# makezur/super_primitive

Measured on AMD Instinct MI355X. Metric: GN iters/sec (640x480x64-seg frame pairs), higher is better.
Workload: dtype f32; 1 GPU; Replica-shaped two-frame SfM, 640x480, 64 segments (grid, 4 px overlap), pyramid level 0 of a 3-level pyramid; BASELINE.json configs[1]; pairs_per_gpu=384, segment_pixels_per_pair=373056, optimiser=gn, tile_points=8192, span_points=4096, granule=64

## Files before the change

include/sp_hip.h:

```cpp
#ifndef SP_HIP_H
#define SP_HIP_H

#include <stdint.h>

#ifdef __cplusplus
extern "C" {
#endif

#define SP_ABI_VERSION 17

#define SP_EINVAL (-1)
#define SP_ELIMIT (-2)

#define SP_GRAD_PARTIAL_FLOATS 16
#define SP_GN_PARTIAL_FLOATS   32
#define SP_GNA_PARTIAL_FLOATS  48

int sp_abi_version(void);


int sp_mask_count(const uint8_t* masks, int N, int H, int W, int32_t* row_counts, int32_t* counts,
                  int32_t* seg_off, void* stream);

int sp_table_fill(const uint8_t* masks, const float* logdepth, const float* keypoints, int N, int H, int W,
// ... 113 lines not shown
#define SP_COST_WAVE_SPANS 0x100
#define SP_COST_DEPTH_TABLE 0x200

int sp_pairs_cost(const SpPair* pairs, const int32_t* chunks, const int32_t* spans, int n_spans, int mode, float irls_eps,
                  float* span_partials, float* seg_partials, void* stream);

int sp_pairs_adam_step(const SpPair* pairs, int n_pairs, int max_N, const float* span_partials, const float* seg_partials,
                       float lr_kld, float lr_pose, float lr_aff, float* state, float* losses, void* stream);

#define SP_LM_STATE_FLOATS 8
int sp_pairs_gn_step(const SpPair* pairs, int n_pairs, int max_N, const float* span_partials, const float* seg_partials,
                     float lm_up, float lm_down, float lm_min, float* lm_state, float* backup, float* costs, void* stream);

int sp_pairs_cost_active(const SpPair* pairs, const int32_t* chunks, const int32_t* spans, int n_spans, int mode, float irls_eps,
                         float* span_partials, float* seg_partials, const int32_t* done, void* stream);
int sp_pairs_gn_step_conv(const SpPair* pairs, int n_pairs, int max_N, const float* span_partials, const float* seg_partials,
                          float lm_up, float lm_down, float lm_min, float* lm_state, float* backup, float* costs, float conv_tol,
                          int32_t* done, void* stream);

#define SP_MAX_PHASES 12
#define SP_PHASE_POSE_ONLY 1
#define SP_PHASE_WAVE_SPANS 2
#define SP_PHASE_DEPTH_TABLE 4
#define SP_PHASE_DEPTH_DAMP_SHIFT 8
#define SP_PHASE_DEPTH_DAMP(k) (((k) & 0xff) << SP_PHASE_DEPTH_DAMP_SHIFT)
#define SP_PHASE_ADAM 8
#define SP_PHASE_PREDICTED_EXIT 16
typedef struct SpPhase {
    const SpPair* pairs;
    const int32_t* chunks;
// ... 272 lines not shown
```

super_primitive_amd/_lib.py:

```python
from __future__ import annotations

import ctypes
import os
from ctypes import c_float, c_int, c_void_p

_HERE = os.path.dirname(os.path.abspath(__file__))
LIB_PATH = os.environ.get("SP_HIP_LIB") or os.path.join(_HERE, "csrc", "libsp_hip.so")

P = c_void_p
I = c_int
F = c_float

SIGNATURES = {
    "sp_abi_version": [],
    "sp_mask_count": [P, I, I, I, P, P, P, P],
    "sp_table_fill": [P, P, P, I, I, I, P, P, P, P, P, P],
    "sp_table_sample_source": [P, P, P, P, P, I, I, I, I, P, I, I, P, P, I, P],
    "sp_pack_rgb": [P, I, I, I, P, P],
    "sp_blur_decimate": [P, I, I, I, P, P],
    "sp_photo_cost_grad": [P, P, P, P, P, P, I, I, I, I, I, P, P, P, I, I, P, P, I, P, P, F, P, P, P, P, P, P],
    "sp_points_workspace_floats": [I, I],
    "sp_points_cost_grad": [P, P, I, I, I, I, P, I, I, P, P, I, P, P, F, P, P, P, P, P],
    "sp_photo_stats": [P, P, P, P, I, I, I, I, P, P, P, I, I, P, P, I, P, P, F, P, P, P, P, P, P, P, P, I, P],
    "sp_pairs_cost": [P, P, P, I, I, F, P, P, P],
    "sp_pairs_adam_step": [P, I, I, P, P, F, F, F, P, P, P],
    "sp_pairs_gn_step": [P, I, I, P, P, F, F, F, P, P, P, P],
    "sp_pairs_cost_active": [P, P, P, I, I, F, P, P, P, P],
    "sp_pairs_gn_step_conv": [P, I, I, P, P, F, F, F, P, P, P, F, P, P],
    "sp_prepare_count": [P, I, I, I, P],
    "sp_prepare_count_boxed": [P, I, I, I, P],
    "sp_prepare_fill": [P, I, I, I, P],
    "sp_prepare_sample": [P, I, I, P],
    "sp_prepare_sample_pairs": [P, I, P, I, I, P],
    "sp_prepare_blur": [P, I, I, I, P],
    "sp_prepare_pack": [P, I, I, P],
    "sp_prepare_blur_pack": [P, I, I, P],
    "sp_prepare_gather": [P, P, I, P, P],
    "sp_host_work_list_chunks": [P, I, I, I],
    "sp_host_layout": [P, I, I, P, I, I, P, P, P, P, P],
    "sp_host_work_list": [P, P, P, I, I, I, I, I, P, P, P, P, P, P],
    "sp_pairs_schedule_cost": [P, P, P],
    "sp_pairs_schedule_gn_step": [P, I, I, F, F, F, P, P, P, P, P, P, P],
# ... 253 lines not shown
```

super_primitive_amd/csrc/sp_cost.hip:

```cpp
#include "sp_solve_device.h"

namespace {

struct TileCtx {
    gptr_u32 pix;
    gptr_f4 src4;
    gptr_f32 trg;
    Cam Ks;
    Warp w;
    float shift;
    float gain, bias;
    float ax, ay;
    uint32_t row_bytes;
    int Wl, Hl;
    int start, count;
};

struct Geo {
    float qx, qy, qz;
    float zinv, zi;
    float px, py, pz;
};

struct Pending {
// ... 239 lines not shown
    f32x2 hd01;
    f32x2 hd[2];
    float h11;
    f32x2 D, bd;
    float cost, n;
    float cost_mark, n_mark;
};

struct Pending2 {
    f32x2 qxy; float qz, zinv, zi;
    f32x2 wxy; float m;
    f32x2 srg; float sb;
    uint32_t off0;
};

template <bool DT = false>
__device__ __forceinline__ void prepare2(const TileCtx& c, const PairConsts& k, float shift, uint32_t pw, const f32x4 s, Pending2& p) {
    const f32x2 colrow{(float)(pw & 0xffffu), (float)((pw >> 16) & 0x7fffu)};
    const bool src_ok = (int32_t)pw < 0;
    const float d = DT ? s.w * shift : fast_exp(s.w + shift);
    const f32x2 xy = pfma(colrow, k.ifxy, k.nKc) * d;
    const f32x2 qxy = pfma(k.R03, f32x2{xy.x, xy.x}, pfma(k.R14, f32x2{xy.y, xy.y}, pfma(k.R25, f32x2{d, d}, k.t01)));
    const float qz = fmaf(k.R6, xy.x, fmaf(k.R7, xy.y, fmaf(k.R8, d, k.t2)));
    const bool zguard = fabsf(qz) > 1e-6f;
    const float zinv = zguard ? __builtin_amdgcn_rcpf(qz) : 1e-6f;
    const f32x2 uv = qxy * k.Kf * zinv + k.Ktc;
    const f32x2 n = pfma(uv, k.invWH, f32x2{-1.f, -1.f});
    const bool ok = (fabsf(n.x) <= 0.99f) && (fabsf(n.y) <= 0.99f) && (qz > k.zmin) && src_ok && (d > 1e-7f);
    p.m = ok ? 1.f : 0.f;
    p.qxy = qxy; p.qz = qz;
    p.zinv = ok ? zinv : 0.f;
    p.zi = (ok && zguard) ? zinv : 0.f;
    p.srg = f32x2{s.x, s.y}; p.sb = s.z;
    const f32x2 ixy = pfma(n, k.sxy, k.sxy);
    const f32x2 fl{floorf(ixy.x), floorf(ixy.y)};
// ... 170 lines not shown
        float v[10] = {A.hd01.x, A.hd01.y, A.hd[0].x, A.hd[0].y, A.hd[1].x, A.hd[1].y, A.D.x + A.D.y, A.bd.x + A.bd.y,
                       A.cost - A.cost_mark, A.n - A.n_mark};
        wave_sum_to_lanes<10>(v, lane, pos, ok);
        if (ok) store_partial<WT>(rec + pos, v[0]);
        A.cost_mark = A.cost; A.n_mark = A.n;
    }
    const f32x2 z{0.f, 0.f};
    A.hd01 = z; A.hd[0] = z; A.hd[1] = z; A.D = z; A.bd = z;
}

__device__ __forceinline__ uint32_t pix_from_colour_bits(const f32x4 s) {
    const uint32_t a = __builtin_bit_cast(uint32_t, s.x), b = __builtin_bit_cast(uint32_t, s.y), c = __builtin_bit_cast(uint32_t, s.z);
    const uint32_t v = (a & 0x7fu) | ((b & 0x7fu) << 7) | ((c & 0x3fu) << 14);
    return (v & 0x3ffu) | (((v >> 10) & 0x1ffu) << 16) | ((v >> 19) << 31);
}
template <int ABL, bool WT, bool AFF = false, bool W64 = false>
__device__ __forceinline__ void run_span_gn(const TileCtx& c, const SpPair& pr, const int4* __restrict__ chunks, int q0,
                                            int n_chunks, int total, float irls_eps, float* __restrict__ span_rec,
                                            float* __restrict__ seg_partials, float* lds) {
    constexpr int TRIP = W64 ? 64 : SP_BLOCK;
    constexpr bool DT = ABL == 6;
    constexpr int NV = AFF ? SP_GNA_PARTIAL_FLOATS : SP_GN_PARTIAL_FLOATS, NS = AFF ? SP_GNA_SEG_FLOATS : SP_GN_SEG_FLOATS;
    GnAcc A;
    AffAcc AA;
    MixA ma{f32x2{0.f, 0.f}, f32x2{0.f, 0.f}};
    {
        const f32x2 z{0.f, 0.f};
        AA.haa = AA.hab = AA.hbb = AA.ba = AA.bb = AA.hda = AA.hdb = 0.f;
        AA.pa01 = z; AA.pb01 = z; AA.pa[0] = z; AA.pa[1] = z; AA.pb[0] = z; AA.pb[1] = z;
    }
    {
        const f32x2 z{0.f, 0.f};
        A.h00 = z; A.bp01 = z; A.hd01 = z;
#pragma unroll
// ... 16 lines not shown
        kc.t01 = f32x2{w.t[0], w.t[1]};        kc.Kf = sgpr2(w.Kt.fx, w.Kt.fy);     kc.Ktc = sgpr2(w.Kt.cx, w.Kt.cy);
        kc.invWH = sgpr2(2.f * w.invWm1, 2.f * w.invHm1);  kc.sxy = sgpr2(w.sx, w.sy);
        kc.gab = sgpr2(c.gain * c.ax * w.Kt.fx, c.gain * c.ay * w.Kt.fy);
        kc.bias2 = f32x2{c.bias, c.bias};      kc.eps2 = sgpr2(irls_eps, irls_eps);
        kc.R6 = sgpr(w.R[6]); kc.R7 = sgpr(w.R[7]); kc.R8 = sgpr(w.R[8]); kc.t2 = w.t[2];
        asm volatile("" : "+v"(kc.nKc), "+v"(kc.bias2), "+v"(kc.t01), "+v"(kc.t2));
        kc.gain = sgpr(c.gain); kc.bias = sgpr(c.bias); kc.zmin = sgpr(w.zmin); kc.eps = sgpr(irls_eps);
        kc.row_bytes_f = sgpr((float)(c.Wl * (int)(4u * SP_TEXEL_FLOATS)));
    }
    const rsrc_t r_pix = make_rsrc(c.pix + start, (uint32_t)total * 4u);
    const rsrc_t r_src = make_rsrc(c.src4 + start, (uint32_t)total * 16u);
    const rsrc_t r_trg = make_rsrc(c.trg, (uint32_t)c.Wl * (uint32_t)c.Hl * (4u * SP_TEXEL_FLOATS));
    const int n_iter = total / TRIP;
    uint32_t op = (W64 ? (threadIdx.x & 63u) : threadIdx.x) * 4u;
    constexpr int NT = 2;
    struct Slot { Pending2 p; int q; bool last; };
    Slot S0, S1;
    {
        const f32x4 s = buf_load4<NT>(r_src, op * 4u);
        const uint32_t pw = ABL == 5 ? pix_from_colour_bits(s) : (uint32_t)__builtin_amdgcn_raw_buffer_load_b32(r_pix, (int)op, 0, NT);
        prepare2<DT>(c, kc, k.shift, pw, s, S0.p);
        S0.last = cursor_advance<TRIP, DT>(k, S0.q);
    }
    S1.p = S0.p;
    S1.p.zinv = 0.f; S1.p.zi = 0.f;
    S1.q = q0; S1.last = false;
    Mix2 m{f32x2{0.f, 0.f}, f32x2{0.f, 0.f}, f32x2{0.f, 0.f}};
    auto trip = [&](Slot& a, Slot& b) {
        op += 4u * TRIP;
        asm volatile("" : "+v"(op));
        const uint32_t pw = ABL == 5 ? 0u : (uint32_t)__builtin_amdgcn_raw_buffer_load_b32(r_pix, (int)op, 0, NT);
        const f32x4 s = buf_load4<NT>(r_src, op * 4u);
        f32x3 ta, tb, tc, td;
        if (ABL == 1) { ta = tb = tc = td = f32x3{a.p.srg.x, a.p.srg.y, a.p.sb}; }
        else if (ABL == 3) {
            const uint32_t lin = (op >> 2) * (4u * SP_TEXEL_FLOATS);
            const uint32_t cap = (uint32_t)(c.Wl * (c.Hl - 2)) * (4u * SP_TEXEL_FLOATS);
            const uint32_t o0 = lin < cap ? lin : lin - cap * (lin / cap);
            ta = buf_load3(r_trg, o0);
            tb = buf_load3(r_trg, o0 + 4u * SP_TEXEL_FLOATS);
            tc = buf_load3(r_trg, o0, c.row_bytes);
            td = buf_load3(r_trg, o0 + 4u * SP_TEXEL_FLOATS, c.row_bytes);
        } else if (ABL == 4) {
            ta = buf_load3(r_trg, a.p.off0);
            tc = buf_load3(r_trg, a.p.off0, c.row_bytes);
            tb = ta; td = tc;
        } else {
// ... 2 lines not shown
            tc = buf_load3(r_trg, a.p.off0, c.row_bytes);
            td = buf_load3(r_trg, a.p.off0 + 4u * SP_TEXEL_FLOATS, c.row_bytes);
        }
        __builtin_amdgcn_sched_barrier(0);
        if (ABL != 2) fold_gn2<AFF>(kc, GeoGn{b.p.qxy, b.p.qz, b.p.zinv, b.p.zi}, m, A, &ma, &AA);
        if (b.last) flush_segment_gn<WT, AFF>(A, seg_partials + (size_t)(W64 ? b.q : 4 * b.q + wave) * NS, &AA);
        __builtin_amdgcn_sched_barrier(0);
        if (ABL != 1)
            asm volatile("" : "+v"(ta), "+v"(tb), "+v"(tc), "+v"(td), "+v"(A.blk[0]), "+v"(A.blk[1]), "+v"(A.blk[2]),
                         "+v"(A.blk[3]), "+v"(A.blk[4]), "+v"(A.blk[5]), "+v"(A.bp[0]), "+v"(A.bp[1]), "+v"(A.hd[0]),
                         "+v"(A.hd[1]), "+v"(A.D), "+v"(A.bd), "+v"(A.h00), "+v"(A.h0[0]), "+v"(A.h0[1]), "+v"(A.h1[0]), "+v"(A.h1[1]), "+v"(A.h11), "+v"(A.bp01), "+v"(A.hd01));
        if (ABL == 2) A.cost += ta.x + tb.y + tc.z + td.x + a.p.wxy.x + a.p.wxy.y + a.p.m;
        else finish_gn2<AFF>(kc, a.p, ta, tb, tc, td, m, A.cost, A.n, &ma, &AA);
        uint32_t pw_ = pw;
        f32x4 s_ = s;
        asm volatile("" : "+v"(pw_), "+v"(s_));
        if (ABL == 5) pw_ = pix_from_colour_bits(s_);
        prepare2<DT>(c, kc, k.shift, pw_, s_, b.p);
        b.last = cursor_advance<TRIP, DT>(k, b.q);
    };
    int j = 0;
    for (; j + 1 < n_iter; j += 2) { trip(S0, S1); trip(S1, S0); }
    if (j < n_iter) {
        trip(S0, S1);
        if (ABL != 2) fold_gn2<AFF>(kc, GeoGn{S0.p.qxy, S0.p.qz, S0.p.zinv, S0.p.zi}, m, A, &ma, &AA);
        flush_segment_gn<WT, AFF>(A, seg_partials + (size_t)(W64 ? S0.q : 4 * S0.q + wave) * NS, &AA);
    } else {
        if (ABL != 2) fold_gn2<AFF>(kc, GeoGn{S1.p.qxy, S1.p.qz, S1.p.zinv, S1.p.zi}, m, A, &ma, &AA);
        flush_segment_gn<WT, AFF>(A, seg_partials + (size_t)(W64 ? S1.q : 4 * S1.q + wave) * NS, &AA);
    }
    float acc[NV];
    acc[0] = A.cost;
    acc[1] = A.h00.x; acc[2] = A.h00.y;
// ... 13 lines not shown
        acc[46] = acc[47] = 0.f;
    } else {
        acc[29] = acc[30] = acc[31] = 0.f;
    }
    if (W64) {
        int pos; bool ok;
        wave_sum_to_lanes<NV>(acc, (int)((op >> 2) & 63u), pos, ok);
        if (ok) store_partial<WT>(span_rec + pos, acc[0]);
    } else {
        const int tid = (int)((op >> 2) & (uint32_t)(SP_BLOCK - 1));
        const float tot = block_sum_to_thread<NV>(acc, lds, tid);
        if (tid < NV) store_partial<WT>(span_rec + tid, tot);
    }
}

template <int ABL, bool WT, bool W64 = false>
__device__ __forceinline__ void run_span_grad(const TileCtx& c, const SpPair& pr, const int4* __restrict__ chunks, int q0,
                                              int n_chunks, int total, float* __restrict__ span_rec,
                                              float* __restrict__ seg_partials, float* lds) {
    constexpr int TRIP = W64 ? 64 : SP_BLOCK;
    constexpr bool DT = ABL == 6;
    constexpr int NV = SP_GRAD_PARTIAL_FLOATS;
    float acc[NV];
#pragma unroll
    for (int i = 0; i < NV; ++i) acc[i] = 0.f;
    const int wave = __builtin_amdgcn_readfirstlane((int)(threadIdx.x >> 6));
    SpanCursor k;
    cursor_init<TRIP, DT>(k, pr, chunks, q0, n_chunks);
    const int start = k.chunks[q0].start;
    const float ifx = 1.f / c.Ks.fx, ify = 1.f / c.Ks.fy;
    const rsrc_t r_pix = make_rsrc(c.pix + start, (uint32_t)total * 4u);
    const rsrc_t r_src = make_rsrc(c.src4 + start, (uint32_t)total * 16u);
    const rsrc_t r_trg = make_rsrc(c.trg, (uint32_t)c.Wl * (uint32_t)c.Hl * (4u * SP_TEXEL_FLOATS));
    const int n_iter = total / TRIP;
    uint32_t op = (W64 ? (threadIdx.x & 63u) : threadIdx.x) * 4u;
    constexpr int NT = 2;
    struct Slot { Pending p; int q; bool last; };
    Slot S0, S1;
    {
        const uint32_t pw = (uint32_t)__builtin_amdgcn_raw_buffer_load_b32(r_pix, (int)op, 0, NT);
        const f32x4 s = buf_load4<NT>(r_src, op * 4u);
        prepare<DT>(c, k.shift, ifx, ify, pw, s, S0.p);
        S0.last = cursor_advance<TRIP, DT>(k, S0.q);
    }
    S1.p = S0.p;
    S1.p.g.zinv = 0.f; S1.p.g.zi = 0.f;
    S1.q = q0; S1.last = false;
    Mix0 m0{0.f, 0.f, 0.f, 0.f};
    auto flush = [&](int q) {
        const float tot = wave_sum(acc[13]);
        if (lane_id() == 0) store_partial<WT>(seg_partials + (size_t)(W64 ? q : 4 * q + wave) * SP_GRAD_SEG_FLOATS, tot);
        acc[13] = 0.f;
    };
    auto trip = [&](Slot& a, Slot& b) {
        op += 4u * TRIP;
        asm volatile("" : "+v"(op));
        const uint32_t pw = (uint32_t)__builtin_amdgcn_raw_buffer_load_b32(r_pix, (int)op, 0, NT);
        const f32x4 s = buf_load4<NT>(r_src, op * 4u);
        f32x3 ta, tb, tc, td;
        if (ABL == 1) { ta = tb = tc = td = f32x3{a.p.sr, a.p.sg, a.p.sb}; }
        else {
            ta = buf_load3(r_trg, a.p.off0);
            tb = buf_load3(r_trg, a.p.off0 + 4u * SP_TEXEL_FLOATS);
            tc = buf_load3(r_trg, a.p.off0, c.row_bytes);
            td = buf_load3(r_trg, a.p.off0 + 4u * SP_TEXEL_FLOATS, c.row_bytes);
        }
        __builtin_amdgcn_sched_barrier(0);
        if (ABL != 2) fold_grad(c, b.p.g, m0, acc);
        if (b.last) flush(b.q);
        __builtin_amdgcn_sched_barrier(0);
        if (ABL != 1)
            asm volatile("" : "+v"(ta), "+v"(tb), "+v"(tc), "+v"(td), "+v"(acc[1]), "+v"(acc[2]), "+v"(acc[3]), "+v"(acc[4]), "+v"(acc[5]),
                         "+v"(acc[6]), "+v"(acc[7]), "+v"(acc[8]), "+v"(acc[9]), "+v"(acc[10]), "+v"(acc[11]), "+v"(acc[12]),
                         "+v"(acc[13]), "+v"(acc[14]), "+v"(acc[15]));
        if (ABL == 2) acc[0] += ta.x + tb.y + tc.z + td.x + a.p.wx + a.p.wy + a.p.m;
        else finish_grad(c, a.p, ta, tb, tc, td, m0, acc[0]);
        uint32_t pw_ = pw;
        f32x4 s_ = s;
        asm volatile("" : "+v"(pw_), "+v"(s_));
        prepare<DT>(c, k.shift, ifx, ify, pw_, s_, b.p);
        b.last = cursor_advance<TRIP, DT>(k, b.q);
    };
    int j = 0;
    for (; j + 1 < n_iter; j += 2) { trip(S0, S1); trip(S1, S0); }
    if (j < n_iter) {
        trip(S0, S1);
        if (ABL != 2) fold_grad(c, S0.p.g, m0, acc);
        flush(S0.q);
    } else {
        if (ABL != 2) fold_grad(c, S1.p.g, m0, acc);
        flush(S1.q);
    }
    if (W64) {
        int pos; bool ok;
        wave_sum_to_lanes<NV>(acc, (int)((op >> 2) & 63u), pos, ok);
// ... 129 lines not shown
    uint32_t mask;
    int32_t vspans;
    int32_t n_lists;
    SchedList list[SP_SCHED_LISTS];
};
struct FuseArgs {
    int32_t* arrivals;
    AdamArgs adam;
    GnArgs gn;
    const int32_t* done;
    const int32_t* phase;
    SchedCost sched;
    const int32_t* active;
    const MultiList* multi;
    int32_t n_multi;
};

template <int MODE, int ABL = 0, int FUSED = 0, bool W64 = false>
__global__ __launch_bounds__(SP_BLOCK, FUSED != 0 ? 1 : (MODE == 2 ? 2 : 4)) void k_cost_pairs(
        const SpPair* __restrict__ pairs, const int4* __restrict__ chunks, const int4* __restrict__ spans, int n_spans,
        float irls_eps, float* __restrict__ partials, float* __restrict__ seg_partials, FuseArgs f) {
    constexpr int NV = MODE == 0 ? SP_GRAD_PARTIAL_FLOATS : (MODE == 2 ? SP_GNA_PARTIAL_FLOATS : SP_GN_PARTIAL_FLOATS);
    __shared__ float lds[SP_WAVES * NV];
    int block = blockIdx.x;
    uint32_t phase_mask = f.sched.mask;
    int vspans = f.sched.vspans;
    if (f.multi) {
        int l = 0;
        for (int i = 1; i < f.n_multi && block >= f.multi[i].first_block; ++i) l = i;
        const MultiList& ml = f.multi[l];
        block -= ml.first_block;
        pairs = ml.pairs; chunks = reinterpret_cast<const int4*>(ml.chunks); spans = reinterpret_cast<const int4*>(ml.spans);
        n_spans = ml.n_spans; partials = ml.partials; seg_partials = ml.seg_partials;
// ... 39 lines not shown
    const SpPair& pr = pairs[owner];
    TileCtx c;
    c.pix = (gptr_u32)pr.pix;
    c.src4 = (gptr_f4)pr.src4;
    c.trg = (gptr_f32)pr.trg3;
    c.Ks = Cam{pr.K_src[0], pr.K_src[1], pr.K_src[2], pr.K_src[3]};
    const Cam Kt{pr.K_trg[0], pr.K_trg[1], pr.K_trg[2], pr.K_trg[3]};
    fill_warp(c, pr.pose, Kt, pr.H, pr.W, pr.Hl, pr.Wl, pr.zmin);
    c.shift = 0.f;
    c.gain = 1.f; c.bias = 0.f;
    if (pr.aff) {
        c.gain = sgpr(expf(-(pr.aff[2] - pr.aff[0])));
        c.bias = sgpr(pr.aff[3] - pr.aff[1]);
    }
    c.start = 0; c.count = 0;
    if (MODE == 2) run_span_gn<ABL, FUSED != 0, true>(c, pr, chunks, span.x, span.y, span.z, irls_eps, partials + (size_t)w * NV, seg_partials, lds);
    else if (MODE == 1) run_span_gn<ABL, FUSED != 0, false, W64>(c, pr, chunks, span.x, span.y, span.z, irls_eps, partials + (size_t)w * NV, seg_partials, lds);
    else run_span_grad<ABL, FUSED != 0, W64>(c, pr, chunks, span.x, span.y, span.z, partials + (size_t)w * NV, seg_partials, lds);
    if (FUSED != 0) {
        __shared__ int is_last;
        asm volatile("s_waitcnt vmcnt(0)" ::: "memory");
        __syncthreads();
        if (threadIdx.x == 0) {
            const int old = __hip_atomic_fetch_add(f.arrivals + span.w, 1, __ATOMIC_RELAXED, __HIP_MEMORY_SCOPE_AGENT);
            const int last = old == pr.n_tiles - 1;
            if (last) {
                __hip_atomic_store(f.arrivals + span.w, 0, __ATOMIC_RELAXED, __HIP_MEMORY_SCOPE_AGENT);
                __builtin_amdgcn_fence(__ATOMIC_ACQUIRE, "agent");
            }
            is_last = last;
        }
        __syncthreads();
        if (is_last) {
// ... 200 lines not shown
        hipLaunchKernelGGL((k_cost_pairs<1, 6>), dim3(gx), dim3(SP_BLOCK), 0, s, pairs, c4, s4, n_spans, irls_eps, partials, seg_partials, nofuse);
    else if (mode == 18)
        hipLaunchKernelGGL((k_cost_pairs<0, 6>), dim3(gx), dim3(SP_BLOCK), 0, s, pairs, c4, s4, n_spans, irls_eps, partials, seg_partials, nofuse);
    else if (mode == 16)
        hipLaunchKernelGGL((k_cost_pairs<1, 5>), dim3(gx), dim3(SP_BLOCK), 0, s, pairs, c4, s4, n_spans, irls_eps, partials, seg_partials, nofuse);
    else if (mode == 15)
        hipLaunchKernelGGL((k_cost_pairs<1, 4>), dim3(gx), dim3(SP_BLOCK), 0, s, pairs, c4, s4, n_spans, irls_eps, partials, seg_partials, nofuse);
    else if (mode == 12)
        hipLaunchKernelGGL((k_cost_pairs<0, 2>), dim3(gx), dim3(SP_BLOCK), 0, s, pairs, c4, s4, n_spans, irls_eps, partials, seg_partials, nofuse);
    else
        hipLaunchKernelGGL((k_cost_pairs<1, 2>), dim3(gx), dim3(SP_BLOCK), 0, s, pairs, c4, s4, n_spans, irls_eps, partials, seg_partials, nofuse);
    SP_CHECK_LAUNCH();
    return 0;
}

}

int cost_pairs_multi(const MultiList* lists_dev, int n_lists, int total_blocks, int mode, float irls_eps, void* stream) {
    if (!lists_dev || n_lists <= 0 || total_blocks <= 0 || (mode != 0 && mode != 1 && mode != 2)) return SP_EINVAL;
    FuseArgs f{};
    f.multi = lists_dev; f.n_multi = n_lists;
    hipStream_t s = static_cast<hipStream_t>(stream);
    const SpPair* np = nullptr; const int4* n4 = nullptr; float* nf = nullptr;
    if (mode == 2) hipLaunchKernelGGL(k_cost_pairs<2>, dim3(total_blocks), dim3(SP_BLOCK), 0, s, np, n4, n4, 0, irls_eps, nf, nf, f);
    else if (mode == 1) hipLaunchKernelGGL(k_cost_pairs<1>, dim3(total_blocks), dim3(SP_BLOCK), 0, s, np, n4, n4, 0, irls_eps, nf, nf, f);
    else hipLaunchKernelGGL(k_cost_pairs<0>, dim3(total_blocks), dim3(SP_BLOCK), 0, s, np, n4, n4, 0, irls_eps, nf, nf, f);
    SP_CHECK_LAUNCH();
    return 0;
}

// ... 120 lines not shown
```

super_primitive_amd/csrc/sp_table.hip:

```cpp
#include "sp_device.h"

namespace {

__device__ __forceinline__ void row_count(const uint8_t* __restrict__ masks, int row, int H, int W, int stride,
                                          int32_t* __restrict__ row_counts) {
    const int lane = threadIdx.x & 63;
    const uint8_t* m = masks + (size_t)row * W;
    int c = 0;
    if (stride == 1) {
        for (int x = lane; x < W; x += 64) c += m[x] != 0;
    } else if ((row % H) % stride == 0) {
        for (int x = lane * stride; x < W; x += 64 * stride) c += m[x] != 0;
    }
#pragma unroll
    for (int o = 32; o > 0; o >>= 1) c += __shfl_xor(c, o, 64);
    if (lane == 0) row_counts[row] = c;
}

__global__ __launch_bounds__(SP_BLOCK) void k_row_counts(const uint8_t* __restrict__ masks, int rows_total, int H, int W,
                                                         int32_t* __restrict__ row_counts) {
    const int row = blockIdx.x * SP_WAVES + (threadIdx.x >> 6);
    if (row >= rows_total) return;
    row_count(masks, row, H, W, 1, row_counts);
}
// ... 1346 lines not shown
int sp_prepare_pack(const SpPrepImage* jobs, int n_jobs, int max_pixels, void* stream) {
    if (!jobs || check_grid(max_pixels, n_jobs)) return SP_EINVAL;
    hipLaunchKernelGGL(k_prep_pack, dim3((max_pixels + SP_BLOCK - 1) / SP_BLOCK, n_jobs), dim3(SP_BLOCK), 0, static_cast<hipStream_t>(stream), jobs);
    SP_CHECK_LAUNCH();
    return 0;
}

int sp_prepare_gather(const float* const* src, const long long* off, int n, float* out, void* stream) {
    if (!src || !off || !out || n <= 0) return SP_EINVAL;
    hipLaunchKernelGGL(k_prep_gather, dim3(n), dim3(64), 0, static_cast<hipStream_t>(stream), src, off, out);
    SP_CHECK_LAUNCH();
    return 0;
}

}
```

super_primitive_amd/optim/pair_batch.py:

```python
from __future__ import annotations

import ctypes

import numpy as np
import torch

from .. import _lib
from ..image import gaussian_pyramid
from . import batch_prepare

_SP_PAIR_DTYPE = np.dtype(_lib.SpPair)

DEFAULT_BATCH_TILE_POINTS = 8192
DEFAULT_SPAN_POINTS = 16384
MIN_SPANS = 2304
GRANULE = 256

FRAME_PAIR_POINT_STRIDE = (2, 2, 4)
FRAME_PAIR_SCHEDULE = dict(max_iters_per_level=25, conv_tol=2e-3, polish_max=15, polish_eps=1e-5, polish_tol=1e-4, check_every=3, predicted_exit=True)
FIXED_FRAME_PAIR_SCHEDULE = dict(iters_per_level=15, polish_iters=10, polish_eps=1e-5)
REFERENCE_START_LEVELS = (0, 3)
REFERENCE_START_POINT_STRIDE = (2, 2, 4)
REFERENCE_START_RETRY = (dict(level=2, stride=4, max_iters=30, irls_eps=1e-3, conv_tol=2e-3, pose_only=True),)
REFERENCE_START_ADAM = (dict(level=2, stride=4, max_iters=500, irls_eps=1e-5, conv_tol=0.0, adam=True),
# ... 72 lines not shown

class _Lazy(dict):

    def __init__(self, make, *a, **kw):
        super().__init__(*a, **kw)
        self._make = make

    def __missing__(self, key):
        self[key] = v = self._make(key)
        return v


class PairBatch:
    def __init__(self, src_frames, trg_images, trg_Ks, poses, klds, levels=(0, 3), use_affine=False,
                 tile_points=DEFAULT_BATCH_TILE_POINTS, zmin=1e-7, replicate=1, span_points=None, point_stride=None,
                 extra_tables=(), lazy_levels=True, timer=None, granule=GRANULE, depth_table=True):
        assert granule in (GRANULE, 64)
        self.granule = int(granule)
        self.rec_per_chunk = 4 if granule == GRANULE else 1
        self.wave_flag = 0 if granule == GRANULE else _lib.SP_COST_WAVE_SPANS
        self.depth_table = bool(depth_table)
        self.table_flag = _lib.SP_COST_DEPTH_TABLE if self.depth_table else 0
        lib = _lib.load()
        self.lib = lib
        M0 = len(src_frames)
        R = int(replicate)
        M = M0 * R
        assert M0 == len(trg_images) == len(trg_Ks) and len(klds) in (M0, M) and poses.shape[0] in (M0, M)
        if poses.shape[0] == M0 and R > 1:
            poses = poses.repeat(R, 1, 1)
        dev = src_frames[0].image.device
# ... 154 lines not shown
        self.adam_state = state_f[cuts[1]: cuts[1] + M * widths[1]].view(M, widths[1])
        self.lm_state = state_f[cuts[2]: cuts[2] + M * widths[2]].view(M, widths[2])
        self.backup = state_f[cuts[3]: cuts[3] + M * widths[3]].view(M, widths[3])
        state_i = torch.zeros(4, M, dtype=torch.int32, device=dev)
        self.arrivals = state_i[0]
        self.done = state_i[1]
        self.phase = state_i[2]
        self.phase_iters = state_i[3]
        mark('workspaces')
        self.reset_lm()
        self._graphs = {}
        self._flags_more = []
        self._flag = None
        self._verdict_arrays = None
        self.status = None
        self._initial = (self.pose.clone(), self.kld.clone())
        mark('constructor returns')

    @property
    def setup_bytes(self):
        if callable(self._setup_bytes):
            self._setup_bytes = self._setup_bytes()
        return self._setup_bytes

    @property
    def seg_records(self):
        return torch.repeat_interleave(self.chunks[:, :2], self.rec_per_chunk, dim=0)

    def restore_initial(self):
        self.pose.copy_(self._initial[0])
# ... 12 lines not shown
        dev = torch.device(device)
        t = lambda a: torch.from_numpy(np.ascontiguousarray(a)).to(dev)
        src = [KeyFrame(t(p.src_image), t(p.K), t(p.logdepth_perseg), t(p.keypoints), t(p.keypoint_regions)) for p in pairs]
        return cls(src, [t(p.trg_image) for p in pairs], [t(p.K) for p in pairs],
                   torch.stack([t(p.pose_init) for p in pairs]), [t(p.kld_init) for p in pairs], levels=levels, **kw)

    def reset_lm(self, lam=1e-4):
        self._lam0 = float(lam)
        self.lm_state.zero_()
        self.lm_state[:, 0] = lam
        self.lm_state[:, 1] = -1.0

    def cost_pass(self, level, mode, irls_eps=1e-3):
        if mode not in (0, 1) and self.table_flag:
            raise ValueError("cost mode 2 and the developer modes read log-depth tables: build the batch with depth_table=False")
        _lib.check(self.lib.sp_pairs_cost(_lib.ptr(self.desc[level]), _lib.ptr(self.chunks), _lib.ptr(self.spans), self.n_spans, mode | self.wave_flag | (self.table_flag if mode in (0, 1) else 0),
                                          float(irls_eps), _lib.ptr(self.partials), _lib.ptr(self.seg_partials), _lib.stream_ptr()), "sp_pairs_cost")

    def gn_step(self, level=0, irls_eps=1e-3, lm_up=8.0, lm_down=0.5, lm_min=1e-7, fused=False, conv_tol=0.0):
        if fused:
            assert not self.wave_flag and not self.table_flag, "the single-launch form has no wave-span / depth-table variant (PairBatch(depth_table=False))"
            _lib.check(self.lib.sp_pairs_gn_iterate(_lib.ptr(self.desc[level]), _lib.ptr(self.chunks), _lib.ptr(self.spans), self.n_spans, self.M,
                                                    self.max_N, float(irls_eps), _lib.ptr(self.partials), _lib.ptr(self.seg_partials), _lib.ptr(self.arrivals),
                                                    float(lm_up), float(lm_down), float(lm_min), _lib.ptr(self.lm_state),
                                                    _lib.ptr(self.backup), _lib.ptr(self._costs), _lib.stream_ptr()),
                       "sp_pairs_gn_iterate")
            return self._costs
        if conv_tol > 0.0:
            _lib.check(self.lib.sp_pairs_cost_active(_lib.ptr(self.desc[level]), _lib.ptr(self.chunks), _lib.ptr(self.spans), self.n_spans, 1 | self.wave_flag | self.table_flag,
                                                     float(irls_eps), _lib.ptr(self.partials), _lib.ptr(self.seg_partials),
                                                     _lib.ptr(self.done), _lib.stream_ptr()), "sp_pairs_cost_active")
            _lib.check(self.lib.sp_pairs_gn_step_conv(_lib.ptr(self.desc[level]), self.M, self.max_N, _lib.ptr(self.partials),
                                                      _lib.ptr(self.seg_partials), float(lm_up), float(lm_down), float(lm_min),
                                                      _lib.ptr(self.lm_state), _lib.ptr(self.backup), _lib.ptr(self._costs),
                                                      float(conv_tol), _lib.ptr(self.done), _lib.stream_ptr()), "sp_pairs_gn_step_conv")
            return self._costs
        self.cost_pass(level, 1, irls_eps)
        return self.solve_gn(level, lm_up, lm_down, lm_min)

    def solve_gn(self, level=0, lm_up=8.0, lm_down=0.5, lm_min=1e-7):
        _lib.check(self.lib.sp_pairs_gn_step(_lib.ptr(self.desc[level]), self.M, self.max_N, _lib.ptr(self.partials), _lib.ptr(self.seg_partials),
                                             float(lm_up), float(lm_down), float(lm_min), _lib.ptr(self.lm_state),
                                             _lib.ptr(self.backup), _lib.ptr(self._costs), _lib.stream_ptr()),
                   "sp_pairs_gn_step")
        return self._costs

# ... 447 lines not shown
```

Before: 451,100 iters/s.

## Replace per-pixel coordinate loads with per-wave run descriptors in cost pass

Adds a one-time build kernel that compresses each 64-pixel group's packed coordinates into a small descriptor: a validity mask, up to two contiguous runs with base column/row and offsets. The wave-span depth-table cost kernels then read this uniform descriptor through the constant/scalar path and rebuild column/row from the lane index, instead of issuing a per-lane buffer load of the pixel word each trip. This cuts vector memory traffic and load latency in the hot loop. The path is used only when every group has at most two runs. It adds a few ALU ops per point, a scalar load per trip, and a host sync at construction.

```diff
diff --git a/include/sp_hip.h b/include/sp_hip.h
--- a/include/sp_hip.h
+++ b/include/sp_hip.h
@@ -151,6 +151,21 @@
 
 int sp_pairs_cost_active(const SpPair* pairs, const int32_t* chunks, const int32_t* spans, int n_spans, int mode, float irls_eps,
                          float* span_partials, float* seg_partials, const int32_t* done, void* stream);
+
+typedef struct SpRunDesc {
+    uint32_t valid[2];
+    float d[2];
+    float base[2];
+    float k;
+    int32_t runs;
+} SpRunDesc;
+
+int sp_run_desc_build(const uint32_t* pix, int n_groups, SpRunDesc* desc, int32_t* n_general, void* stream);
+int sp_pairs_cost_rd(const SpPair* pairs, const int32_t* chunks, const int32_t* spans, int n_spans, int mode, float irls_eps,
+                     float* span_partials, float* seg_partials, const uint32_t* pix_base, const SpRunDesc* desc, void* stream);
+int sp_pairs_cost_rd_active(const SpPair* pairs, const int32_t* chunks, const int32_t* spans, int n_spans, int mode, float irls_eps,
+                            float* span_partials, float* seg_partials, const int32_t* done, const uint32_t* pix_base,
+                            const SpRunDesc* desc, void* stream);
 int sp_pairs_gn_step_conv(const SpPair* pairs, int n_pairs, int max_N, const float* span_partials, const float* seg_partials,
                           float lm_up, float lm_down, float lm_min, float* lm_state, float* backup, float* costs, float conv_tol,
                           int32_t* done, void* stream);
diff --git a/super_primitive_amd/_lib.py b/super_primitive_amd/_lib.py
--- a/super_primitive_amd/_lib.py
+++ b/super_primitive_amd/_lib.py
@@ -26,6 +26,9 @@
     "sp_pairs_adam_step": [P, I, I, P, P, F, F, F, P, P, P],
     "sp_pairs_gn_step": [P, I, I, P, P, F, F, F, P, P, P, P],
     "sp_pairs_cost_active": [P, P, P, I, I, F, P, P, P, P],
+    "sp_run_desc_build": [P, I, P, P, P],
+    "sp_pairs_cost_rd": [P, P, P, I, I, F, P, P, P, P, P],
+    "sp_pairs_cost_rd_active": [P, P, P, I, I, F, P, P, P, P, P, P],
     "sp_pairs_gn_step_conv": [P, I, I, P, P, F, F, F, P, P, P, F, P, P],
     "sp_prepare_count": [P, I, I, I, P],
     "sp_prepare_count_boxed": [P, I, I, I, P],
diff --git a/super_primitive_amd/csrc/sp_cost.hip b/super_primitive_amd/csrc/sp_cost.hip
--- a/super_primitive_amd/csrc/sp_cost.hip
+++ b/super_primitive_amd/csrc/sp_cost.hip
@@ -277,11 +277,52 @@
     uint32_t off0;
 };
 
+__device__ __forceinline__ void prepare2_at(const PairConsts& k, f32x2 colrow, bool src_ok, float d, const f32x4 s, Pending2& p);
+
 template <bool DT = false>
 __device__ __forceinline__ void prepare2(const TileCtx& c, const PairConsts& k, float shift, uint32_t pw, const f32x4 s, Pending2& p) {
     const f32x2 colrow{(float)(pw & 0xffffu), (float)((pw >> 16) & 0x7fffu)};
     const bool src_ok = (int32_t)pw < 0;
     const float d = DT ? s.w * shift : fast_exp(s.w + shift);
+    prepare2_at(k, colrow, src_ok, d, s, p);
+}
+
+typedef const SpRunDesc __attribute__((address_space(4)))* cptr_rd;
+__device__ __forceinline__ SpRunDesc rd_load(cptr_rd p) {
+    SpRunDesc r;
+    r.valid[0] = p->valid[0]; r.valid[1] = p->valid[1];
+    r.d[0] = p->d[0]; r.d[1] = p->d[1];
+    r.base[0] = p->base[0]; r.base[1] = p->base[1];
+    r.k = p->k; r.runs = p->runs;
+    return r;
+}
+__device__ __forceinline__ f32x2 rd_colrow(const SpRunDesc& r, f32x2 lane2) {
+    const float step = __builtin_amdgcn_fmed3f(lane2.x + r.k, 0.f, 1.f);
+    return pfma(step, f32x2{r.d[0], r.d[1]}, lane2) + f32x2{r.base[0], r.base[1]};
+}
+__device__ __forceinline__ float rd_depth(const SpRunDesc& r, float d) {
+    const uint64_t m = ((uint64_t)r.valid[1] << 32) | r.valid[0];
+    float o;
+    asm("v_cndmask_b32_e64 %0, 0, %1, %2" : "=v"(o) : "v"(d), "s"(m));
+    return o;
+}
+template <bool DT>
+__device__ __forceinline__ void prepare2_rd(const PairConsts& k, float shift, const SpRunDesc& r, f32x2 lane2, const f32x4 s, Pending2& p) {
+    const f32x2 colrow = rd_colrow(r, lane2);
+    const float d = rd_depth(r, DT ? s.w * shift : fast_exp(s.w + shift));
+    prepare2_at(k, colrow, true, d, s, p);
+}
+template <bool DT>
+__device__ __forceinline__ void prepare_rd(const TileCtx& c, float shift, float ifx, float ify, const SpRunDesc& r, f32x2 lane2, const f32x4 s,
+                                           Pending& p) {
+    const f32x2 colrow = rd_colrow(r, lane2);
+    const float d = rd_depth(r, DT ? s.w * shift : fast_exp(s.w + shift));
+    float x, y;
+    backproject(colrow.x, colrow.y, d, c.Ks, ifx, ify, x, y);
+    prepare_xyz(c, x, y, d, true, s.x, s.y, s.z, p);
+}
+
+__device__ __forceinline__ void prepare2_at(const PairConsts& k, f32x2 colrow, bool src_ok, float d, const f32x4 s, Pending2& p) {
     const f32x2 xy = pfma(colrow, k.ifxy, k.nKc) * d;
     const f32x2 qxy = pfma(k.R03, f32x2{xy.x, xy.x}, pfma(k.R14, f32x2{xy.y, xy.y}, pfma(k.R25, f32x2{d, d}, k.t01)));
     const float qz = fmaf(k.R6, xy.x, fmaf(k.R7, xy.y, fmaf(k.R8, d, k.t2)));
@@ -482,10 +523,11 @@
     const uint32_t v = (a & 0x7fu) | ((b & 0x7fu) << 7) | ((c & 0x3fu) << 14);
     return (v & 0x3ffu) | (((v >> 10) & 0x1ffu) << 16) | ((v >> 19) << 31);
 }
-template <int ABL, bool WT, bool AFF = false, bool W64 = false>
+template <int ABL, bool WT, bool AFF = false, bool W64 = false, bool RD = false>
 __device__ __forceinline__ void run_span_gn(const TileCtx& c, const SpPair& pr, const int4* __restrict__ chunks, int q0,
                                             int n_chunks, int total, float irls_eps, float* __restrict__ span_rec,
-                                            float* __restrict__ seg_partials, float* lds) {
+                                            float* __restrict__ seg_partials, float* lds, const SpRunDesc* rd = nullptr) {
+    static_assert(!RD || (W64 && ABL == 6 && !AFF), "run descriptors: wave spans on depth tables");
     constexpr int TRIP = W64 ? 64 : SP_BLOCK;
     constexpr bool DT = ABL == 6;
     constexpr int NV = AFF ? SP_GNA_PARTIAL_FLOATS : SP_GN_PARTIAL_FLOATS, NS = AFF ? SP_GNA_SEG_FLOATS : SP_GN_SEG_FLOATS;
@@ -532,12 +574,18 @@
     const int n_iter = total / TRIP;
     uint32_t op = (W64 ? (threadIdx.x & 63u) : threadIdx.x) * 4u;
     constexpr int NT = 2;
+    cptr_rd rg = (cptr_rd)rd + (start >> 6);
+    f32x2 lane2{(float)(threadIdx.x & 63u), 0.f};
+    if (RD) asm volatile("" : "+v"(lane2));
     struct Slot { Pending2 p; int q; bool last; };
     Slot S0, S1;
     {
         const f32x4 s = buf_load4<NT>(r_src, op * 4u);
-        const uint32_t pw = ABL == 5 ? pix_from_colour_bits(s) : (uint32_t)__builtin_amdgcn_raw_buffer_load_b32(r_pix, (int)op, 0, NT);
-        prepare2<DT>(c, kc, k.shift, pw, s, S0.p);
+        if (RD) prepare2_rd<DT>(kc, k.shift, rd_load(rg), lane2, s, S0.p);
+        else {
+            const uint32_t pw = ABL == 5 ? pix_from_colour_bits(s) : (uint32_t)__builtin_amdgcn_raw_buffer_load_b32(r_pix, (int)op, 0, NT);
+            prepare2<DT>(c, kc, k.shift, pw, s, S0.p);
+        }
         S0.last = cursor_advance<TRIP, DT>(k, S0.q);
     }
     S1.p = S0.p;
@@ -547,8 +595,10 @@
     auto trip = [&](Slot& a, Slot& b) {
         op += 4u * TRIP;
         asm volatile("" : "+v"(op));
-        const uint32_t pw = ABL == 5 ? 0u : (uint32_t)__builtin_amdgcn_raw_buffer_load_b32(r_pix, (int)op, 0, NT);
+        const uint32_t pw = (ABL == 5 || RD) ? 0u : (uint32_t)__builtin_amdgcn_raw_buffer_load_b32(r_pix, (int)op, 0, NT);
         const f32x4 s = buf_load4<NT>(r_src, op * 4u);
+        SpRunDesc rn;
+        if (RD) { ++rg; rn = rd_load(rg); }
         f32x3 ta, tb, tc, td;
         if (ABL == 1) { ta = tb = tc = td = f32x3{a.p.srg.x, a.p.srg.y, a.p.sb}; }
         else if (ABL == 3) {
@@ -581,9 +631,11 @@
         else finish_gn2<AFF>(kc, a.p, ta, tb, tc, td, m, A.cost, A.n, &ma, &AA);
         uint32_t pw_ = pw;
         f32x4 s_ = s;
-        asm volatile("" : "+v"(pw_), "+v"(s_));
+        if (RD) asm volatile("" : "+v"(s_));
+        else asm volatile("" : "+v"(pw_), "+v"(s_));
         if (ABL == 5) pw_ = pix_from_colour_bits(s_);
-        prepare2<DT>(c, kc, k.shift, pw_, s_, b.p);
+        if (RD) prepare2_rd<DT>(kc, k.shift, rn, lane2, s_, b.p);
+        else prepare2<DT>(c, kc, k.shift, pw_, s_, b.p);
         b.last = cursor_advance<TRIP, DT>(k, b.q);
     };
     int j = 0;
@@ -627,10 +679,11 @@
     }
 }
 
-template <int ABL, bool WT, bool W64 = false>
+template <int ABL, bool WT, bool W64 = false, bool RD = false>
 __device__ __forceinline__ void run_span_grad(const TileCtx& c, const SpPair& pr, const int4* __restrict__ chunks, int q0,
                                               int n_chunks, int total, float* __restrict__ span_rec,
-                                              float* __restrict__ seg_partials, float* lds) {
+                                              float* __restrict__ seg_partials, float* lds, const SpRunDesc* rd = nullptr) {
+    static_assert(!RD || (W64 && ABL == 6), "run descriptors: wave spans on depth tables");
     constexpr int TRIP = W64 ? 64 : SP_BLOCK;
     constexpr bool DT = ABL == 6;
     constexpr int NV = SP_GRAD_PARTIAL_FLOATS;
@@ -648,12 +701,18 @@
     const int n_iter = total / TRIP;
     uint32_t op = (W64 ? (threadIdx.x & 63u) : threadIdx.x) * 4u;
     constexpr int NT = 2;
+    cptr_rd rg = (cptr_rd)rd + (start >> 6);
+    f32x2 lane2{(float)(threadIdx.x & 63u), 0.f};
+    if (RD) asm volatile("" : "+v"(lane2));
     struct Slot { Pending p; int q; bool last; };
     Slot S0, S1;
     {
-        const uint32_t pw = (uint32_t)__builtin_amdgcn_raw_buffer_load_b32(r_pix, (int)op, 0, NT);
         const f32x4 s = buf_load4<NT>(r_src, op * 4u);
-        prepare<DT>(c, k.shift, ifx, ify, pw, s, S0.p);
+        if (RD) prepare_rd<DT>(c, k.shift, ifx, ify, rd_load(rg), lane2, s, S0.p);
+        else {
+            const uint32_t pw = (uint32_t)__builtin_amdgcn_raw_buffer_load_b32(r_pix, (int)op, 0, NT);
+            prepare<DT>(c, k.shift, ifx, ify, pw, s, S0.p);
+        }
         S0.last = cursor_advance<TRIP, DT>(k, S0.q);
     }
     S1.p = S0.p;
@@ -668,8 +727,10 @@
     auto trip = [&](Slot& a, Slot& b) {
         op += 4u * TRIP;
         asm volatile("" : "+v"(op));
-        const uint32_t pw = (uint32_t)__builtin_amdgcn_raw_buffer_load_b32(r_pix, (int)op, 0, NT);
+        const uint32_t pw = RD ? 0u : (uint32_t)__builtin_amdgcn_raw_buffer_load_b32(r_pix, (int)op, 0, NT);
         const f32x4 s = buf_load4<NT>(r_src, op * 4u);
+        SpRunDesc rn;
+        if (RD) { ++rg; rn = rd_load(rg); }
         f32x3 ta, tb, tc, td;
         if (ABL == 1) { ta = tb = tc = td = f32x3{a.p.sr, a.p.sg, a.p.sb}; }
         else {
@@ -690,8 +751,10 @@
         else finish_grad(c, a.p, ta, tb, tc, td, m0, acc[0]);
         uint32_t pw_ = pw;
         f32x4 s_ = s;
-        asm volatile("" : "+v"(pw_), "+v"(s_));
-        prepare<DT>(c, k.shift, ifx, ify, pw_, s_, b.p);
+        if (RD) asm volatile("" : "+v"(s_));
+        else asm volatile("" : "+v"(pw_), "+v"(s_));
+        if (RD) prepare_rd<DT>(c, k.shift, ifx, ify, rn, lane2, s_, b.p);
+        else prepare<DT>(c, k.shift, ifx, ify, pw_, s_, b.p);
         b.last = cursor_advance<TRIP, DT>(k, b.q);
     };
     int j = 0;
@@ -851,9 +914,11 @@
     const int32_t* active;
     const MultiList* multi;
     int32_t n_multi;
+    const uint32_t* rd_pix;
+    const SpRunDesc* rd_desc;
 };
 
-template <int MODE, int ABL = 0, int FUSED = 0, bool W64 = false>
+template <int MODE, int ABL = 0, int FUSED = 0, bool W64 = false, bool RD = false>
 __global__ __launch_bounds__(SP_BLOCK, FUSED != 0 ? 1 : (MODE == 2 ? 2 : 4)) void k_cost_pairs(
         const SpPair* __restrict__ pairs, const int4* __restrict__ chunks, const int4* __restrict__ spans, int n_spans,
         float irls_eps, float* __restrict__ partials, float* __restrict__ seg_partials, FuseArgs f) {
@@ -923,9 +988,10 @@
         c.bias = sgpr(pr.aff[3] - pr.aff[1]);
     }
     c.start = 0; c.count = 0;
+    const SpRunDesc* rd = RD ? f.rd_desc + ((const uint32_t*)pr.pix - f.rd_pix) / 64 : nullptr;
     if (MODE == 2) run_span_gn<ABL, FUSED != 0, true>(c, pr, chunks, span.x, span.y, span.z, irls_eps, partials + (size_t)w * NV, seg_partials, lds);
-    else if (MODE == 1) run_span_gn<ABL, FUSED != 0, false, W64>(c, pr, chunks, span.x, span.y, span.z, irls_eps, partials + (size_t)w * NV, seg_partials, lds);
-    else run_span_grad<ABL, FUSED != 0, W64>(c, pr, chunks, span.x, span.y, span.z, partials + (size_t)w * NV, seg_partials, lds);
+    else if (MODE == 1) run_span_gn<ABL, FUSED != 0, false, W64, RD>(c, pr, chunks, span.x, span.y, span.z, irls_eps, partials + (size_t)w * NV, seg_partials, lds, rd);
+    else run_span_grad<ABL, FUSED != 0, W64, RD>(c, pr, chunks, span.x, span.y, span.z, partials + (size_t)w * NV, seg_partials, lds, rd);
     if (FUSED != 0) {
         __shared__ int is_last;
         asm volatile("s_waitcnt vmcnt(0)" ::: "memory");
@@ -1156,6 +1222,33 @@
     return 0;
 }
 
+int sp_pairs_cost_rd_active(const SpPair* pairs, const int32_t* chunks, const int32_t* spans, int n_spans, int mode, float irls_eps,
+                            float* partials, float* seg_partials, const int32_t* done, const uint32_t* pix_base, const SpRunDesc* desc,
+                            void* stream) {
+    if (!pairs || !chunks || !spans || !partials || !seg_partials || !pix_base || !desc || n_spans <= 0) return SP_EINVAL;
+    const int base = mode & ~(SP_COST_WAVE_SPANS | SP_COST_DEPTH_TABLE);
+    if (!(mode & SP_COST_WAVE_SPANS) || !(mode & SP_COST_DEPTH_TABLE) || (base != 0 && base != 1)) return SP_EINVAL;
+    hipStream_t s = static_cast<hipStream_t>(stream);
+    const int gw = ((((n_spans + 3) / 4) + 7) / 8) * 8;
+    FuseArgs f{};
+    f.done = done;
+    f.rd_pix = pix_base;
+    f.rd_desc = desc;
+    const int4* c4 = reinterpret_cast<const int4*>(chunks);
+    const int4* s4 = reinterpret_cast<const int4*>(spans);
+    if (base == 0)
+        hipLaunchKernelGGL((k_cost_pairs<0, 6, 0, true, true>), dim3(gw), dim3(SP_BLOCK), 0, s, pairs, c4, s4, n_spans, irls_eps, partials, seg_partials, f);
+    else
+        hipLaunchKernelGGL((k_cost_pairs<1, 6, 0, true, true>), dim3(gw), dim3(SP_BLOCK), 0, s, pairs, c4, s4, n_spans, irls_eps, partials, seg_partials, f);
+    SP_CHECK_LAUNCH();
+    return 0;
+}
+
+int sp_pairs_cost_rd(const SpPair* pairs, const int32_t* chunks, const int32_t* spans, int n_spans, int mode, float irls_eps,
+                     float* partials, float* seg_partials, const uint32_t* pix_base, const SpRunDesc* desc, void* stream) {
+    return sp_pairs_cost_rd_active(pairs, chunks, spans, n_spans, mode, irls_eps, partials, seg_partials, nullptr, pix_base, desc, stream);
+}
+
 }
 
 int cost_pairs_multi(const MultiList* lists_dev, int n_lists, int total_blocks, int mode, float irls_eps, void* stream) {
diff --git a/super_primitive_amd/csrc/sp_table.hip b/super_primitive_amd/csrc/sp_table.hip
--- a/super_primitive_amd/csrc/sp_table.hip
+++ b/super_primitive_amd/csrc/sp_table.hip
@@ -1384,3 +1384,42 @@
 }
 
 }
+
+__global__ __launch_bounds__(SP_BLOCK) void k_run_desc_build(const uint32_t* __restrict__ pix, int n_groups, SpRunDesc* __restrict__ desc,
+                                                             int32_t* __restrict__ n_general) {
+    const int g = blockIdx.x * SP_WAVES + (int)(threadIdx.x >> 6);
+    if (g > n_groups) return;
+    const int lane = (int)(threadIdx.x & 63u);
+    const uint32_t w = g < n_groups ? pix[(size_t)g * 64 + lane] : 0u;
+    const uint32_t v = w & 0x7fffffffu;
+    const uint64_t valid = __ballot((w >> 31) != 0u);
+    const uint64_t nz = __ballot(w != 0u);
+    const int last = nz ? 63 - __clzll((long long)nz) : 0;
+    const uint32_t prev = (uint32_t)__shfl_up((int)v, 1);
+    const uint64_t starts = __ballot(lane == 0 || (lane <= last && v != prev + 1u));
+    const int runs = __popcll(starts);
+    const uint64_t rest = starts & ~1ull;
+    const int s1 = rest ? __ffsll((long long)rest) - 1 : 64;
+    const uint32_t v0 = (uint32_t)__shfl((int)v, 0), v1 = (uint32_t)__shfl((int)v, s1 & 63);
+    const int c0 = (int)(v0 & 0xffffu), r0 = (int)(v0 >> 16);
+    const int c1 = s1 < 64 ? (int)(v1 & 0xffffu) : c0 + s1, r1 = s1 < 64 ? (int)(v1 >> 16) : r0;
+    const int f = lane & 7;
+    const uint32_t word = f == 0 ? (uint32_t)valid : f == 1 ? (uint32_t)(valid >> 32)
+                        : f == 2 ? __float_as_uint((float)(c1 - s1 - c0)) : f == 3 ? __float_as_uint((float)(r1 - r0))
+                        : f == 4 ? __float_as_uint((float)c0) : f == 5 ? __float_as_uint((float)r0)
+                        : f == 6 ? __float_as_uint((float)(1 - s1)) : (uint32_t)runs;
+    if (lane < 8) reinterpret_cast<uint32_t*>(desc + g)[lane] = word;
+    if (lane == 0 && runs > 2 && g < n_groups) atomicAdd(n_general, 1);
+}
+
+extern "C" {
+
+int sp_run_desc_build(const uint32_t* pix, int n_groups, SpRunDesc* desc, int32_t* n_general, void* stream) {
+    if (!pix || !desc || !n_general || n_groups <= 0) return SP_EINVAL;
+    const int blocks = (n_groups + 1 + SP_WAVES - 1) / SP_WAVES;
+    hipLaunchKernelGGL(k_run_desc_build, dim3(blocks), dim3(SP_BLOCK), 0, static_cast<hipStream_t>(stream), pix, n_groups, desc, n_general);
+    SP_CHECK_LAUNCH();
+    return 0;
+}
+
+}
diff --git a/super_primitive_amd/optim/pair_batch.py b/super_primitive_amd/optim/pair_batch.py
--- a/super_primitive_amd/optim/pair_batch.py
+++ b/super_primitive_amd/optim/pair_batch.py
@@ -110,7 +110,7 @@
 class PairBatch:
     def __init__(self, src_frames, trg_images, trg_Ks, poses, klds, levels=(0, 3), use_affine=False,
                  tile_points=DEFAULT_BATCH_TILE_POINTS, zmin=1e-7, replicate=1, span_points=None, point_stride=None,
-                 extra_tables=(), lazy_levels=True, timer=None, granule=GRANULE, depth_table=True):
+                 extra_tables=(), lazy_levels=True, timer=None, granule=GRANULE, depth_table=True, run_desc=True):
         assert granule in (GRANULE, 64)
         self.granule = int(granule)
         self.rec_per_chunk = 4 if granule == GRANULE else 1
@@ -295,6 +295,15 @@
         self._flag = None
         self._verdict_arrays = None
         self.status = None
+        self.run_desc = None
+        if run_desc and self.granule == 64 and self.depth_table:
+            n_groups = self.pix.numel() // 64
+            rd = torch.empty((n_groups + 1) * 8, dtype=torch.int32, device=dev)
+            n_general = torch.zeros(1, dtype=torch.int32, device=dev)
+            _lib.check(lib.sp_run_desc_build(_lib.ptr(self.pix), n_groups, _lib.ptr(rd), _lib.ptr(n_general), _lib.stream_ptr()), "sp_run_desc_build")
+            if int(n_general.item()) == 0:
+                self.run_desc = rd
+            mark('run descriptors')
         self._initial = (self.pose.clone(), self.kld.clone())
         mark('constructor returns')
 
@@ -337,6 +346,11 @@
     def cost_pass(self, level, mode, irls_eps=1e-3):
         if mode not in (0, 1) and self.table_flag:
             raise ValueError("cost mode 2 and the developer modes read log-depth tables: build the batch with depth_table=False")
+        if self.run_desc is not None and mode in (0, 1):
+            _lib.check(self.lib.sp_pairs_cost_rd(_lib.ptr(self.desc[level]), _lib.ptr(self.chunks), _lib.ptr(self.spans), self.n_spans, mode | self.wave_flag | self.table_flag,
+                                                 float(irls_eps), _lib.ptr(self.partials), _lib.ptr(self.seg_partials), _lib.ptr(self.pix),
+                                                 _lib.ptr(self.run_desc), _lib.stream_ptr()), "sp_pairs_cost_rd")
+            return
         _lib.check(self.lib.sp_pairs_cost(_lib.ptr(self.desc[level]), _lib.ptr(self.chunks), _lib.ptr(self.spans), self.n_spans, mode | self.wave_flag | (self.table_flag if mode in (0, 1) else 0),
                                           float(irls_eps), _lib.ptr(self.partials), _lib.ptr(self.seg_partials), _lib.stream_ptr()), "sp_pairs_cost")
 
@@ -350,9 +364,15 @@
                        "sp_pairs_gn_iterate")
             return self._costs
         if conv_tol > 0.0:
-            _lib.check(self.lib.sp_pairs_cost_active(_lib.ptr(self.desc[level]), _lib.ptr(self.chunks), _lib.ptr(self.spans), self.n_spans, 1 | self.wave_flag | self.table_flag,
-                                                     float(irls_eps), _lib.ptr(self.partials), _lib.ptr(self.seg_partials),
-                                                     _lib.ptr(self.done), _lib.stream_ptr()), "sp_pairs_cost_active")
+            if self.run_desc is not None:
+                _lib.check(self.lib.sp_pairs_cost_rd_active(_lib.ptr(self.desc[level]), _lib.ptr(self.chunks), _lib.ptr(self.spans), self.n_spans,
+                                                            1 | self.wave_flag | self.table_flag, float(irls_eps), _lib.ptr(self.partials),
+                                                            _lib.ptr(self.seg_partials), _lib.ptr(self.done), _lib.ptr(self.pix), _lib.ptr(self.run_desc),
+                                                            _lib.stream_ptr()), "sp_pairs_cost_rd_active")
+            else:
+                _lib.check(self.lib.sp_pairs_cost_active(_lib.ptr(self.desc[level]), _lib.ptr(self.chunks), _lib.ptr(self.spans), self.n_spans, 1 | self.wave_flag | self.table_flag,
+                                                         float(irls_eps), _lib.ptr(self.partials), _lib.ptr(self.seg_partials),
+                                                         _lib.ptr(self.done), _lib.stream_ptr()), "sp_pairs_cost_active")
             _lib.check(self.lib.sp_pairs_gn_step_conv(_lib.ptr(self.desc[level]), self.M, self.max_N, _lib.ptr(self.partials),
                                                       _lib.ptr(self.seg_partials), float(lm_up), float(lm_down), float(lm_min),
                                                       _lib.ptr(self.lm_state), _lib.ptr(self.backup), _lib.ptr(self._costs),
```

After: 465,800 iters/s (median of 6 runs). 3.3% higher.
